# ruuda/robigo-luculenta

Hardware: AMD Instinct MI355X
Metric: Mrays/sec on built-in scene at 1920x1080 (higher is better)
Workload: dtype f32

## Files before the change

__graft_entry__.py:

```python
import os
import subprocess
import sys

ROOT = os.path.dirname(os.path.abspath(__file__))


def _make(directory):
    subprocess.run(["make", "-C", os.path.join(ROOT, directory)], check=True)


def build():
    _make("robigo_luculenta_amd/csrc")
    _make("oracle")
    _make("tests/host_mirror")
    _make("tests/lds_poison")
    _make("examples")
    if ROOT not in sys.path:
        sys.path.insert(0, ROOT)
    import robigo_luculenta_amd


def smoke():
    if ROOT not in sys.path:
        sys.path.insert(0, ROOT)
    sys.path.insert(0, os.path.join(ROOT, "tests"))
    import numpy as np

    import robigo_luculenta_amd as R
    import _oracle as O

    assert R.device_count() > 0, "smoke() needs a GPU"
    W, H, N = 256, 144, 16384
    objs, cam = R.builtin_scene_desc(R.SCENE_DEMO)
    scene = R.Scene(objs, cam, device=0)
    trace = R.TraceUnit(0, W, H, n_photons=N)
    trace.render(scene, seed=1, stream=0, first_path_index=0)
    got = trace.mapped_photons
    want, segs = O.Scene(objs.view(O.OBJECT_DTYPE), O.RlCameraDesc.from_buffer_copy(bytes(cam))).render(W, H, 1, 0, 0, N, threads=4)
    assert got.tobytes() == want.tobytes(), "GPU photons differ from the CPU oracle"
    paths, segments, ms = trace.stats()
    assert (paths, segments) == (N, segs), (paths, segments, N, segs)
    plot = R.PlotUnit(0, W, H)
    plot.plot([trace])
    gather = R.GatherUnit(W, H)
    gather.accumulate(plot)
    tm = R.TonemapUnit(W, H)
    tm.tonemap(gather)
    rgb = tm.rgb_buffer
    ref_rgb, _, _ = O.tonemap(gather.tristimulus_buffer, W, H)
    assert np.abs(rgb.astype(int) - ref_rgb.astype(int)).max() <= 1
    print("smoke ok: %d photons bit-equal to the oracle, %d segments, %.3f ms kernel" % (N, segments, ms))


if __name__ == "__main__":
    build()
    if len(sys.argv) > 1 and sys.argv[1] == "smoke":
        smoke()
```

robigo_luculenta_amd/csrc/rl_scene.cpp:

```cpp
#include "rl_scene.h"

#include <algorithm>
#include <array>
#include <cmath>
#include <cstdio>
#include <cstdlib>
#include <cstring>
#include <limits>
#include <numeric>

#include "rl_core.h"

namespace {

const float PI = RL_PI_F;

RlVector3 V(float x, float y, float z) {
    RlVector3 v;
    v.x = x; v.y = y; v.z = z;
    return v;
}
RlVector3 V(RlF3 f) { return V(f.x, f.y, f.z); }
RlF3 F(const RlVector3& v) { return rl_f3(v.x, v.y, v.z); }
RlF4 F4(RlF3 v, float w) {
// ... 50 lines not shown
    for (int i = 0; i < count; ++i) {
        for (int v = 0; v < 2; ++v) {
            const float ofs = variants[v][0], radius = variants[v][1], phi_ofs = variants[v][2], h = variants[v][3];
            const float phi = (float)i * prism_angle + ofs;
            RlF3 position = rl_f3(rl_cosf_d(phi) * prism_radius * radius, rl_sinf_d(phi) * prism_radius * radius, 0.0f);
            RlF3 normal = rl_f3(0, 0, -1.0f);
            const float t = rl_paraboloid_t(floor.offset, floor.normal, floor.focal_point, position, normal);
            if (!(t < 0.0f)) {
                const RlF3 pos = rl_add(position, rl_mul(normal, t));
                const RlF3 local_pos = rl_sub(pos, floor.offset);
                const RlF3 plane_pr = rl_sub(local_pos, rl_mul(floor.normal, rl_dot(local_pos, floor.normal)));
                const RlF3 surface_normal = rl_normalise(rl_sub(floor.focal_point, plane_pr));
                normal = rl_neg(surface_normal);
                position = rl_add(pos, rl_mul(rl_mul(normal, 2.0f), h));
            }
            out.push_back(make_object(RL_SURFACE_HEX_PRISM, V(normal), V(position), 3.0f, 1.0f, phi + phi_ofs, prism_height * h,
                                      RL_MATERIAL_SF10_GLASS, 0, 0, 0));
        }
    }
}

RlCameraDesc demo_camera() {
    RlCameraDesc c;
    c.phi0 = 1.0f; c.phi1 = 0.01f;
    c.alpha0 = 0.3f; c.alpha1 = -0.01f;
    c.dist0 = 50.0f; c.dist1 = -0.5f;
    c.fov_over_pi = 0.35f;
    c.focal_factor = 0.9f;
    c.depth_of_field = 2.0f;
    c.chromatic_abberation = 0.012f;
    return c;
}

void demo_scene(int seeds, std::vector<RlObjectDesc>& out) {
    const float sun_radius = 5.0f;
    push_fixed_objects(out, sun_radius);
    const double golden_ratio = 1.6180339887498948482045868343656381177203091798057628;
    const float gamma = PI * 2.0f * (1.0f - 1.0f / (float)golden_ratio);
    const float seed_size = 0.8f, seed_scale = 1.5f;
    const float fs = sun_radius / seed_scale + 1.0f;
    const int first_seed = (int)(fs * fs + 0.5f);
    for (int i = first_seed; i < first_seed + seeds; ++i) {
        const float phi = (float)i * gamma;
        const float r = sqrtf((float)i) * seed_scale;
        const RlF3 c = rl_add(rl_f3(rl_cosf_d(phi) * r, rl_sinf_d(phi) * r, (r - sun_radius) * -0.5f), rl_f3(0, 0, 0));
        out.push_back(sphere(c, seed_size, RL_MATERIAL_DIFFUSE_COLOURED, 0.9f,
                             (float)(i - first_seed) / (float)seeds * 130.0f + 600.0f, 60.0f));
    }
    for (int i = first_seed; i < first_seed + seeds; ++i) {
        const float fi = (float)i + 0.5f;
        const float phi = fi * gamma;
        const float r = sqrtf(fi) * seed_scale;
        const RlF3 c = rl_add(rl_f3(rl_cosf_d(phi) * r, rl_sinf_d(phi) * r, (r - sun_radius) * -0.25f), rl_f3(0, 0, 0));
        out.push_back(sphere(c, seed_size * 0.5f, RL_MATERIAL_GLOSSY_MIRROR, 0.1f));
    }
    for (int i = first_seed / 2; i < first_seed + seeds; ++i) {
        const float phi = (float)(-i) * gamma;
        const float root = sqrtf((float)i);
        const float r = root * seed_scale * 1.5f;
        const RlF3 c = rl_add(rl_f3(rl_cosf_d(phi) * r, rl_sinf_d(phi) * r, (r - sun_radius) * 1.5f + sun_radius * 2.0f), rl_f3(0, 0, 0));
        out.push_back(sphere(c, seed_size * (0.5f + root * 0.2f), RL_MATERIAL_SOAP_BUBBLE));
    }
    push_prism_ring(out, sun_radius, 11, 17.0f);
}

void glass_stress_scene(std::vector<RlObjectDesc>& out) {
    const float sun_radius = 5.0f;
    push_fixed_objects(out, sun_radius);
    push_prism_ring(out, sun_radius, 11, 10.0f);
    push_prism_ring(out, sun_radius, 11, 17.0f);
    push_prism_ring(out, sun_radius, 11, 24.0f);
}

void push_infinite_prism(std::vector<RlF4>& recs, RlF3 axis, RlF3 offset, float edge_length, float angle, float objbits) {
    const float radius = sqrtf(3.0f) / 6.0f * edge_length;
    const float a[3] = {angle, angle + PI * 2.0f / 3.0f, angle + PI * 4.0f / 3.0f};
    for (int k = 0; k < 3; ++k) {
        const RlF3 p = rl_rotate_towards(rl_f3(rl_cosf_d(a[k]), rl_sinf_d(a[k]), 0.0f), axis);
        recs.push_back(F4(p, 0.0f));
        recs.push_back(F4(rl_add(rl_mul(p, radius), offset), objbits));
    }
}

void prism_vertices(const RlF4* pr, std::vector<double>& vx, std::vector<double>& vy, std::vector<double>& vz) {
    double n[8][3], d[8];
    for (int k = 0; k < 8; ++k) {
        n[k][0] = pr[2 * k].x; n[k][1] = pr[2 * k].y; n[k][2] = pr[2 * k].z;
        d[k] = n[k][0] * pr[2 * k + 1].x + n[k][1] * pr[2 * k + 1].y + n[k][2] * pr[2 * k + 1].z;
    }
    for (int a = 0; a < 8; ++a)
        for (int b = a + 1; b < 8; ++b)
            for (int c = b + 1; c < 8; ++c) {
                const double* A = n[a]; const double* B = n[b]; const double* Cc = n[c];
                const double bxc[3] = {B[1] * Cc[2] - B[2] * Cc[1], B[2] * Cc[0] - B[0] * Cc[2], B[0] * Cc[1] - B[1] * Cc[0]};
                const double cxa[3] = {Cc[1] * A[2] - Cc[2] * A[1], Cc[2] * A[0] - Cc[0] * A[2], Cc[0] * A[1] - Cc[1] * A[0]};
                const double axb[3] = {A[1] * B[2] - A[2] * B[1], A[2] * B[0] - A[0] * B[2], A[0] * B[1] - A[1] * B[0]};
                const double det = A[0] * bxc[0] + A[1] * bxc[1] + A[2] * bxc[2];
                if (std::fabs(det) < 1e-9) continue;
                double p[3];
                for (int i = 0; i < 3; ++i) p[i] = (d[a] * bxc[i] + d[b] * cxa[i] + d[c] * axb[i]) / det;
                bool inside = true;
                for (int k = 0; k < 8 && inside; ++k)
                    inside = (n[k][0] * p[0] + n[k][1] * p[1] + n[k][2] * p[2] - d[k]) <= 1e-6;
                if (inside) {
                    vx.push_back(p[0]); vy.push_back(p[1]); vz.push_back(p[2]);
                }
            }
}

RlF4 prism_bound(const RlF4* pr) {
    std::vector<double> vx, vy, vz;
    prism_vertices(pr, vx, vy, vz);
    bool unbounded = false;
    RlF4 r;
    r.x = r.y = r.z = 0.0f;
    r.w = std::numeric_limits<float>::infinity();
    if (vx.size() < 4) return r;
    double c[3] = {0, 0, 0};
    for (size_t i = 0; i < vx.size(); ++i) { c[0] += vx[i]; c[1] += vy[i]; c[2] += vz[i]; }
    for (int i = 0; i < 3; ++i) c[i] /= (double)vx.size();
    double r2 = 0;
    for (size_t i = 0; i < vx.size(); ++i) {
        const double dx = vx[i] - c[0], dy = vy[i] - c[1], dz = vz[i] - c[2];
        r2 = std::max(r2, dx * dx + dy * dy + dz * dz);
    }
    if (!(r2 < 1e12)) unbounded = true;
    if (unbounded) return r;
    const double radius = std::sqrt(r2) * 1.05 + 1e-3;
    r.x = (float)c[0]; r.y = (float)c[1]; r.z = (float)c[2];
    r.w = (float)(radius * radius);
    return r;
}

void prism_cylinder(const RlF4* pr, RlF4 out[2]) {
    out[0] = RlF4{0.0f, 0.0f, 0.0f, std::numeric_limits<float>::infinity()};
    out[1] = RlF4{0.0f, 0.0f, 1.0f, 0.0f};
    std::vector<double> vx, vy, vz;
    prism_vertices(pr, vx, vy, vz);
    double a[3] = {pr[14].x, pr[14].y, pr[14].z};
    const double al = std::sqrt(a[0] * a[0] + a[1] * a[1] + a[2] * a[2]);
    if (vx.size() < 4 || !(al > 1e-12)) return;
    for (double& v : a) v /= al;
    double c[3] = {0, 0, 0};
    for (size_t i = 0; i < vx.size(); ++i) { c[0] += vx[i]; c[1] += vy[i]; c[2] += vz[i]; }
    for (double& v : c) v /= (double)vx.size();
    double r2 = 0;
    for (size_t i = 0; i < vx.size(); ++i) {
        const double d[3] = {vx[i] - c[0], vy[i] - c[1], vz[i] - c[2]};
        const double along = d[0] * a[0] + d[1] * a[1] + d[2] * a[2];
        r2 = std::max(r2, d[0] * d[0] + d[1] * d[1] + d[2] * d[2] - along * along);
    }
    if (!(r2 < 1e12)) return;
    out[0] = RlF4{(float)c[0], (float)c[1], (float)c[2], (float)(std::sqrt(std::max(r2, 0.0)) * 1.05 + 1e-3)};
    out[1] = RlF4{(float)a[0], (float)a[1], (float)a[2], 0.0f};
}

struct SphereIn {
    RlF4 rec;
    uint32_t obj;
    double radius;
};

void split_clusters(const std::vector<SphereIn>& sph, std::vector<uint32_t> idx, std::vector<std::vector<uint32_t>>& out, size_t K) {
    if (idx.size() <= K) {
        if (!idx.empty()) out.push_back(idx);
        return;
    }
    double lo[3] = {1e300, 1e300, 1e300}, hi[3] = {-1e300, -1e300, -1e300};
    for (uint32_t i : idx) {
        const double c[3] = {sph[i].rec.x, sph[i].rec.y, sph[i].rec.z};
        for (int a = 0; a < 3; ++a) {
            lo[a] = std::min(lo[a], c[a]);
            hi[a] = std::max(hi[a], c[a]);
        }
    }
    int axis = 0;
    for (int a = 1; a < 3; ++a)
        if (hi[a] - lo[a] > hi[axis] - lo[axis]) axis = a;
    auto coord = [&](uint32_t i) { return axis == 0 ? sph[i].rec.x : axis == 1 ? sph[i].rec.y : sph[i].rec.z; };
    std::sort(idx.begin(), idx.end(), [&](uint32_t a, uint32_t b) { return coord(a) < coord(b) || (coord(a) == coord(b) && a < b); });
    size_t left = ((idx.size() / 2 + K - 1) / K) * K;
    if (left >= idx.size()) left = idx.size() - K;
    split_clusters(sph, std::vector<uint32_t>(idx.begin(), idx.begin() + left), out, K);
    split_clusters(sph, std::vector<uint32_t>(idx.begin() + left, idx.end()), out, K);
}

void refine_clusters(const std::vector<SphereIn>& sph, std::vector<std::vector<uint32_t>>& clusters, size_t K) {
    const size_t k = clusters.size();
    if (k < 2) return;
    std::vector<uint32_t> all;
    for (const auto& c : clusters) all.insert(all.end(), c.begin(), c.end());
    std::sort(all.begin(), all.end());
    for (int iteration = 0; iteration < 24; ++iteration) {
        std::vector<double> cx(k, 0), cy(k, 0), cz(k, 0);
        for (size_t j = 0; j < k; ++j) {
            for (uint32_t i : clusters[j]) {
                cx[j] += sph[i].rec.x; cy[j] += sph[i].rec.y; cz[j] += sph[i].rec.z;
            }
            const double n = (double)std::max<size_t>(1, clusters[j].size());
            cx[j] /= n; cy[j] /= n; cz[j] /= n;
        }
        auto dist2 = [&](uint32_t i, size_t j) {
            const double dx = sph[i].rec.x - cx[j], dy = sph[i].rec.y - cy[j], dz = sph[i].rec.z - cz[j];
            return dx * dx + dy * dy + dz * dz;
        };
        std::vector<std::pair<double, uint32_t>> order;
        for (uint32_t i : all) {
            double best = 1e300, second = 1e300;
            for (size_t j = 0; j < k; ++j) {
                const double d = dist2(i, j);
                if (d < best) { second = best; best = d; }
                else if (d < second) second = d;
            }
            order.push_back({std::sqrt(best) - std::sqrt(second), i});
        }
        std::sort(order.begin(), order.end());
        std::vector<std::vector<uint32_t>> next(k);
        for (const auto& entry : order) {
            const uint32_t i = entry.second;
            size_t pick = k;
            double pick_d = 1e300;
            for (size_t j = 0; j < k; ++j) {
                if (next[j].size() >= K) continue;
                const double d = dist2(i, j);
                if (d < pick_d) { pick_d = d; pick = j; }
            }
            next[pick].push_back(i);
        }
        bool same = true;
        for (size_t j = 0; j < k && same; ++j) {
            std::sort(next[j].begin(), next[j].end());
            std::vector<uint32_t> old = clusters[j];
            std::sort(old.begin(), old.end());
            same = old == next[j];
        }
        clusters = next;
        if (same) break;
// ... 35 lines not shown
    return radius * radius;
}
void improve_partition(const std::vector<Ball>& items, std::vector<std::vector<uint32_t>>& bins, size_t capacity) {
    const size_t k = bins.size();
    if (k < 2) return;
    for (const Ball& b : items)
        if (!(b.r < 1e15)) return;
    const size_t NEIGHBOURS = 6, CANDIDATES = 3, PARTNERS = 4;
    std::vector<double> r2(k);
    std::vector<std::array<double, 3>> centre(k);
    auto refresh = [&](size_t j) {
        r2[j] = bin_radius2(items, bins[j]);
        std::array<double, 3> c = {0, 0, 0};
        for (uint32_t i : bins[j])
            for (int a = 0; a < 3; ++a) c[a] += items[i].c[a];
        for (int a = 0; a < 3; ++a) c[a] /= (double)std::max<size_t>(1, bins[j].size());
        centre[j] = c;
    };
    for (size_t j = 0; j < k; ++j) refresh(j);
    auto outermost = [&](size_t j, size_t count) {
        std::vector<std::pair<double, uint32_t>> by_reach;
        for (uint32_t i : bins[j]) {
            double d2 = 0;
            for (int a = 0; a < 3; ++a) d2 += (items[i].c[a] - centre[j][a]) * (items[i].c[a] - centre[j][a]);
            by_reach.push_back({-(std::sqrt(d2) + items[i].r), i});
        }
        std::sort(by_reach.begin(), by_reach.end());
        std::vector<uint32_t> out;
        for (size_t n = 0; n < by_reach.size() && n < count; ++n) out.push_back(by_reach[n].second);
        return out;
    };
    auto without = [](std::vector<uint32_t> v, uint32_t i) {
        v.erase(std::find(v.begin(), v.end(), i));
        return v;
    };
    const int passes = k <= 256 ? 8 : k <= 1024 ? 3 : 1;
    for (int pass = 0; pass < passes; ++pass) {
        bool improved = false;
        for (size_t a = 0; a < k; ++a) {
            if (bins[a].size() < 2) continue;
            for (uint32_t i : outermost(a, CANDIDATES)) {
                std::vector<std::pair<double, size_t>> near;
                for (size_t b = 0; b < k; ++b) {
                    if (b == a || bins[b].empty()) continue;
                    double d2 = 0;
                    for (int x = 0; x < 3; ++x) d2 += (items[i].c[x] - centre[b][x]) * (items[i].c[x] - centre[b][x]);
                    near.push_back({d2, b});
                }
                std::sort(near.begin(), near.end());
                double best_gain = 1e-9 * (r2[a] + 1.0);
                size_t best_b = k;
                std::vector<uint32_t> best_a_members, best_b_members;
                const std::vector<uint32_t> a_less = without(bins[a], i);
                for (size_t n = 0; n < near.size() && n < NEIGHBOURS; ++n) {
                    const size_t b = near[n].second;
                    const double before = r2[a] + r2[b];
                    if (bins[b].size() < capacity) {
                        std::vector<uint32_t> b_more = bins[b];
                        b_more.push_back(i);
                        const double gain = before - (bin_radius2(items, a_less) + bin_radius2(items, b_more));
                        if (gain > best_gain) { best_gain = gain; best_b = b; best_a_members = a_less; best_b_members = b_more; }
                    }
                    for (uint32_t j : outermost(b, PARTNERS)) {
                        std::vector<uint32_t> a_new = a_less, b_new = without(bins[b], j);
                        a_new.push_back(j);
                        b_new.push_back(i);
                        const double gain = before - (bin_radius2(items, a_new) + bin_radius2(items, b_new));
                        if (gain > best_gain) { best_gain = gain; best_b = b; best_a_members = a_new; best_b_members = b_new; }
                    }
                }
                if (best_b == k) continue;
                bins[a] = best_a_members;
                bins[best_b] = best_b_members;
                refresh(a);
                refresh(best_b);
                improved = true;
                break;
            }
        }
        if (!improved) break;
    }
}

RlF4 cluster_bound(const std::vector<SphereIn>& sph, const std::vector<uint32_t>& members) {
    double c[3] = {0, 0, 0};
    for (uint32_t i : members) {
        c[0] += sph[i].rec.x; c[1] += sph[i].rec.y; c[2] += sph[i].rec.z;
    }
    for (int a = 0; a < 3; ++a) c[a] /= (double)members.size();
    auto reach = [&](uint32_t i) {
        const double dx = sph[i].rec.x - c[0], dy = sph[i].rec.y - c[1], dz = sph[i].rec.z - c[2];
        return std::sqrt(dx * dx + dy * dy + dz * dz) + sph[i].radius;
    };
    for (int it = 0; it < 64; ++it) {
        uint32_t far = members[0];
        for (uint32_t i : members)
            if (reach(i) > reach(far)) far = i;
        const double step = 0.5 / (it + 2.0);
        c[0] += (sph[far].rec.x - c[0]) * step; c[1] += (sph[far].rec.y - c[1]) * step; c[2] += (sph[far].rec.z - c[2]) * step;
    }
    double radius = 0;
    for (uint32_t i : members) radius = std::max(radius, reach(i));
    radius = radius * 1.05 + 0.05;
    RlF4 b;
    b.x = (float)c[0]; b.y = (float)c[1]; b.z = (float)c[2];
    b.w = (float)(radius * radius);
    if (!(radius < 1e15)) b.w = std::numeric_limits<float>::infinity();
    return b;
}


double bound_radius(const RlF4& b) { return b.w > 0.0f ? std::sqrt((double)b.w) : 0.0; }

void split_groups(const std::vector<RlF4>& b, std::vector<uint32_t> idx, std::vector<std::vector<uint32_t>>& out, size_t G) {
    if (idx.size() <= G) {
        if (!idx.empty()) out.push_back(idx);
        return;
    }
    double lo[3] = {1e300, 1e300, 1e300}, hi[3] = {-1e300, -1e300, -1e300};
    for (uint32_t i : idx) {
        const double c[3] = {b[i].x, b[i].y, b[i].z};
        for (int a = 0; a < 3; ++a) {
            lo[a] = std::min(lo[a], c[a]);
            hi[a] = std::max(hi[a], c[a]);
        }
    }
    int axis = 0;
    for (int a = 1; a < 3; ++a)
        if (hi[a] - lo[a] > hi[axis] - lo[axis]) axis = a;
    auto coord = [&](uint32_t i) { return axis == 0 ? b[i].x : axis == 1 ? b[i].y : b[i].z; };
    std::sort(idx.begin(), idx.end(), [&](uint32_t p, uint32_t q) { return coord(p) < coord(q) || (coord(p) == coord(q) && p < q); });
    size_t left = ((idx.size() / 2 + G - 1) / G) * G;
    if (left >= idx.size()) left = idx.size() - G;
    split_groups(b, std::vector<uint32_t>(idx.begin(), idx.begin() + left), out, G);
    split_groups(b, std::vector<uint32_t>(idx.begin() + left, idx.end()), out, G);
}

void refine_groups(const std::vector<RlF4>& b, std::vector<std::vector<uint32_t>>& groups, size_t G) {
    const size_t k = groups.size();
    if (k < 2) return;
    std::vector<uint32_t> all;
    for (const auto& g : groups) all.insert(all.end(), g.begin(), g.end());
    std::sort(all.begin(), all.end());
    for (int iteration = 0; iteration < 24; ++iteration) {
        std::vector<double> cx(k, 0), cy(k, 0), cz(k, 0);
        for (size_t j = 0; j < k; ++j) {
            for (uint32_t i : groups[j]) {
                cx[j] += b[i].x; cy[j] += b[i].y; cz[j] += b[i].z;
            }
            const double n = (double)std::max<size_t>(1, groups[j].size());
            cx[j] /= n; cy[j] /= n; cz[j] /= n;
        }
        auto dist2 = [&](uint32_t i, size_t j) {
            const double dx = b[i].x - cx[j], dy = b[i].y - cy[j], dz = b[i].z - cz[j];
            return dx * dx + dy * dy + dz * dz;
        };
        std::vector<std::pair<double, uint32_t>> order;
        for (uint32_t i : all) {
            double best = 1e300, second = 1e300;
            for (size_t j = 0; j < k; ++j) {
                const double d = dist2(i, j);
                if (d < best) { second = best; best = d; }
                else if (d < second) second = d;
            }
            order.push_back({std::sqrt(best) - std::sqrt(second), i});
        }
        std::sort(order.begin(), order.end());
        std::vector<std::vector<uint32_t>> next(k);
        for (const auto& entry : order) {
            const uint32_t i = entry.second;
            size_t pick = k;
            double pick_d = 1e300;
            for (size_t j = 0; j < k; ++j) {
                if (next[j].size() >= G) continue;
                const double d = dist2(i, j);
                if (d < pick_d) { pick_d = d; pick = j; }
            }
            next[pick].push_back(i);
        }
        bool same = true;
        for (size_t j = 0; j < k && same; ++j) {
            std::sort(next[j].begin(), next[j].end());
            std::vector<uint32_t> old = groups[j];
            std::sort(old.begin(), old.end());
            same = old == next[j];
        }
        groups = next;
        if (same) break;
    }
    std::vector<std::vector<uint32_t>> kept;
    for (auto& g : groups)
        if (!g.empty()) kept.push_back(g);
    groups = kept;
}

RlF4 group_bound(const std::vector<RlF4>& b, const std::vector<uint32_t>& members) {
    RlF4 r;
    r.x = r.y = r.z = 0.0f;
    r.w = std::numeric_limits<float>::infinity();
    for (uint32_t i : members)
        if (!(b[i].w < 1e30f)) return r;
    double c[3] = {0, 0, 0};
    for (uint32_t i : members) {
        c[0] += b[i].x; c[1] += b[i].y; c[2] += b[i].z;
    }
    for (int a = 0; a < 3; ++a) c[a] /= (double)members.size();
    auto reach = [&](uint32_t i) {
        const double dx = b[i].x - c[0], dy = b[i].y - c[1], dz = b[i].z - c[2];
        return std::sqrt(dx * dx + dy * dy + dz * dz) + bound_radius(b[i]);
    };
    for (int it = 0; it < 64; ++it) {
        uint32_t far = members[0];
        for (uint32_t i : members)
            if (reach(i) > reach(far)) far = i;
        const double step = 0.5 / (it + 2.0);
        c[0] += (b[far].x - c[0]) * step; c[1] += (b[far].y - c[1]) * step; c[2] += (b[far].z - c[2]) * step;
    }
    r.x = (float)c[0]; r.y = (float)c[1]; r.z = (float)c[2];
    c[0] = r.x; c[1] = r.y; c[2] = r.z;
    double radius = 0;
    for (uint32_t i : members) radius = std::max(radius, reach(i));
    radius = radius * 1.001 + 1e-3;
    r.w = (float)(radius * radius);
    if (!(radius < 1e15)) r.w = std::numeric_limits<float>::infinity();
    return r;
}

std::vector<uint32_t> order_by_groups(const std::vector<RlF4>& bounds, std::vector<std::vector<uint32_t>>* groups_out, size_t G) {
    std::vector<uint32_t> idx(bounds.size());
    std::iota(idx.begin(), idx.end(), 0u);
    std::vector<std::vector<uint32_t>> groups;
    split_groups(bounds, idx, groups, G);
    refine_groups(bounds, groups, G);
    {
        std::vector<Ball> balls;
        for (const RlF4& b : bounds) balls.push_back(Ball{{b.x, b.y, b.z}, bound_radius(b)});
        improve_partition(balls, groups, G);
    }
    std::vector<uint32_t> order;
    for (std::vector<uint32_t>& g : groups) {
        std::sort(g.begin(), g.end());
        order.insert(order.end(), g.begin(), g.end());
    }
    *groups_out = groups;
    return order;
}

constexpr uint32_t RL_SUPER_MIN_GROUPS = 112;
constexpr uint32_t RL_SUPER_G_DEFAULT = 8;
void super_params(uint32_t* min_groups, uint32_t* sg) {
    *min_groups = RL_SUPER_MIN_GROUPS;
    *sg = RL_SUPER_G_DEFAULT;
    if (const char* e = std::getenv("RL_SUPER_MIN")) *min_groups = (uint32_t)std::max(1, std::atoi(e));
    if (const char* e = std::getenv("RL_SUPER_G")) *sg = (uint32_t)std::min(64, std::max(2, std::atoi(e)));
}
struct ClusterPlan {
    uint32_t k, group_gc;
    std::vector<std::vector<uint32_t>> clusters;
    std::vector<RlF4> cluster_bounds, group_bounds;
    double cost;
};

ClusterPlan plan_clusters(const std::vector<SphereIn>& sph, const std::vector<std::vector<uint32_t>>& clusters, uint32_t k, uint32_t group_gc) {
    ClusterPlan plan;
    plan.k = k;
    plan.group_gc = group_gc;
    plan.cost = 0;
    std::vector<RlF4> bounds;
    for (const std::vector<uint32_t>& members : clusters) bounds.push_back(cluster_bound(sph, members));
    std::vector<std::vector<uint32_t>> groups;
    order_by_groups(bounds, &groups, group_gc);
    const RlF4 never = RlF4{0.0f, 0.0f, 0.0f, -std::numeric_limits<float>::infinity()};
    for (const std::vector<uint32_t>& g : groups) {
        std::vector<RlF4> members;
        std::vector<uint32_t> all(g.size());
        for (uint32_t k2 : g) {
            plan.clusters.push_back(clusters[k2]);
            plan.cluster_bounds.push_back(bounds[k2]);
            members.push_back(bounds[k2]);
        }
        std::iota(all.begin(), all.end(), 0u);
        plan.group_bounds.push_back(group_bound(members, all));
        for (size_t pad = g.size(); pad < group_gc; ++pad) {
            plan.clusters.push_back(std::vector<uint32_t>());
            plan.cluster_bounds.push_back(never);
        }
    }
    return plan;
}

std::vector<RlF4> sample_path_rays(const RlFlatScene& fs, const std::vector<SphereIn>& sph) {
    std::vector<RlF4> spheres, objects = fs.objects;
    std::vector<uint32_t> sphere_obj;
    for (const SphereIn& si : sph) {
        objects[si.obj].w = rl_u2f(rl_object_bits(rl_object_surface(rl_f2u(objects[si.obj].w)), rl_object_material(rl_f2u(objects[si.obj].w)), (uint32_t)spheres.size()));
        spheres.push_back(si.rec);
        sphere_obj.push_back(si.obj);
    }
    RlSceneView sv;
    std::memset(&sv, 0, sizeof sv);
    sv.spheres = spheres.data();
    sv.sphere_obj = sphere_obj.data();
    sv.objects = objects.data();
    sv.planes = fs.planes.data();
    sv.parabs = fs.parabs.data();
    sv.prisms = fs.prisms.data();
    sv.n_direct = sv.n_direct_padded = sv.cluster_base = (uint32_t)spheres.size();
    sv.n_planes = (uint32_t)(fs.planes.size() / 2);
    sv.n_parabs = (uint32_t)(fs.parabs.size() / 3);
    sv.n_prisms = (uint32_t)(fs.prisms.size() / RL_PRISM_STRIDE);
    sv.n_objects = (uint32_t)objects.size();
    sv.camera_rec = fs.camera_rec.data();
    RlSceneView flat_things = sv;
    flat_things.n_direct = 0;
    flat_things.n_prisms = 0;
    std::vector<RlF4> rays;
    const uint64_t seed = 0x706c616e6e696e67ull;
    for (uint64_t path = 0; path < 384 && rays.size() < 2 * 2048; ++path) {
        RlPath p;
        rl_begin_path(sv, 16.0f / 9.0f, seed, 0u, path, &p);
        for (int bounce = 0; bounce < 64; ++bounce) {
            const RlHit nearest_flat = rl_scan(flat_things, p.origin, p.direction);
            rays.push_back(RlF4{p.origin.x, p.origin.y, p.origin.z, nearest_flat.t * 1.0002f});
            rays.push_back(RlF4{p.direction.x, p.direction.y, p.direction.z, 0.0f});
            const RlHit hit = rl_scan(sv, p.origin, p.direction);
            float value = 0.0f;
            uint32_t emitter = 0;
            if (rl_bounce(sv, seed, 0u, path, &p, hit, &value, &emitter) != RL_PATH_CONTINUES) break;
        }
    }
    return rays;
}

double plan_cost(const ClusterPlan& plan, const std::vector<RlF4>& rays) {
    auto reaches = [](const RlF4& b, const RlF4& o, const RlF4& d) {
        if (!(b.w > 0.0f)) return false;
        const double cx = (double)b.x - o.x, cy = (double)b.y - o.y, cz = (double)b.z - o.z;
        const double d2 = (double)d.x * d.x + (double)d.y * d.y + (double)d.z * d.z;
        const double along = std::min(std::max(0.0, (cx * d.x + cy * d.y + cz * d.z) / d2), (double)o.w);
        const double px = cx - along * d.x, py = cy - along * d.y, pz = cz - along * d.z;
        return px * px + py * py + pz * pz <= (double)b.w;
    };
    const double n_rays = (double)(rays.size() / 2);
    uint32_t min_groups, sg;
    super_params(&min_groups, &sg);
    const size_t n_groups = plan.group_bounds.size();
    std::vector<std::vector<uint32_t>> supers;
    std::vector<RlF4> super_bounds;
    if (n_groups >= min_groups && n_groups > sg) {
        order_by_groups(plan.group_bounds, &supers, sg);
        for (const std::vector<uint32_t>& members : supers) super_bounds.push_back(group_bound(plan.group_bounds, members));
    } else {
        supers.assign(1, std::vector<uint32_t>());
        for (uint32_t g = 0; g < n_groups; ++g) supers[0].push_back(g);
    }
    double super_pairs = 0, group_pairs = 0, cluster_pairs = 0;
    for (size_t r = 0; r + 1 < rays.size(); r += 2) {
        for (size_t s = 0; s < supers.size(); ++s) {
            if (!super_bounds.empty()) {
                if (!reaches(super_bounds[s], rays[r], rays[r + 1])) continue;
                super_pairs += 1;
            }
            for (uint32_t g : supers[s]) {
                if (!reaches(plan.group_bounds[g], rays[r], rays[r + 1])) continue;
                group_pairs += 1;
                for (size_t k = plan.group_gc * g; k < plan.group_gc * (g + 1); ++k)
                    if (reaches(plan.cluster_bounds[k], rays[r], rays[r + 1])) cluster_pairs += 1;
            }
        }
    }
    const double top = super_bounds.empty() ? 0.59 * (double)n_groups
                                            : 0.59 * (double)super_bounds.size() + super_pairs / n_rays * (2.3 + 0.9 * (double)sg);
    const double cost = top + group_pairs / n_rays * (2.13 + 0.83 * ((double)plan.group_gc - 3.0)) +
                        cluster_pairs / n_rays * (0.25 + 0.40 * plan.k);
    return cost;
}

}

uint32_t rl_builtin_scene(int which, int param, std::vector<RlObjectDesc>* out, RlCameraDesc* camera) {
    std::vector<RlObjectDesc> objs;
    if (which == RL_SCENE_DEMO) demo_scene(param > 0 ? param : 100, objs);
    else if (which == RL_SCENE_GLASS_STRESS) glass_stress_scene(objs);
    else return 0;
    if (camera) *camera = demo_camera();
    if (out) *out = objs;
    return (uint32_t)objs.size();
}

static void set_group(RlF4& object, uint32_t group_index) {
    const uint32_t bits = rl_f2u(object.w);
    object.w = rl_u2f(rl_object_bits(rl_object_surface(bits), rl_object_material(bits), group_index));
}

int rl_flatten_scene(const RlSceneDesc* desc, RlFlatScene* out, const char** err) {
    *err = "";
    if (!desc || (!desc->objects && desc->n_objects)) {
        *err = "null scene description";
        return RL_E_INVALID;
    }
    if (desc->n_objects > (1u << 24)) {
        *err = "more than 2^24 objects";
        return RL_E_INVALID;
    }
    RlFlatScene& fs = *out;
    fs = RlFlatScene();
    std::vector<SphereIn> sph_in;
    fs.camera = desc->camera;
    const float fov = PI * desc->camera.fov_over_pi;
    fs.screen_distance = 1.0f / rl_tanf(fov * 0.5f);
    fs.camera_rec.assign(3, RlF4{0.0f, 0.0f, 0.0f, 0.0f});
    std::memcpy(fs.camera_rec.data(), &fs.camera, sizeof(RlCameraDesc));
    reinterpret_cast<float*>(fs.camera_rec.data())[10] = fs.screen_distance;
    for (uint32_t i = 0; i < desc->n_objects; ++i) {
        const RlObjectDesc& o = desc->objects[i];
        const float objbits = rl_u2f(i);
        uint32_t group_index = 0;
        switch (o.surface_kind) {
        case RL_SURFACE_SPHERE: {
            SphereIn si;
            si.rec = F4(F(o.v0), o.f0 * o.f0);
            si.obj = i;
            si.radius = std::fabs((double)o.f0);
            sph_in.push_back(si);
            group_index = 0;
            break;
        }
        case RL_SURFACE_PLANE:
        case RL_SURFACE_CIRCLE:
            group_index = (uint32_t)(fs.planes.size() / 2);
            fs.planes.push_back(F4(F(o.v0), o.surface_kind == RL_SURFACE_CIRCLE ? o.f0 * o.f0 : -1.0f));
            fs.planes.push_back(F4(F(o.v1), objbits));
            break;
        case RL_SURFACE_PARABOLOID: {
// ... 114 lines not shown
    }
    fs.cluster_k = plan.k;
    fs.group_gc = plan.group_gc;
    {
        uint32_t min_groups, sg;
        super_params(&min_groups, &sg);
        const size_t n_groups = plan.clusters.size() / plan.group_gc;
        if (n_groups >= min_groups && n_groups > sg) {
            std::vector<std::vector<uint32_t>> supers;
            order_by_groups(plan.group_bounds, &supers, sg);
            std::vector<std::vector<uint32_t>> ordered;
            for (const std::vector<uint32_t>& members : supers) {
                for (uint32_t g : members)
                    for (uint32_t c = 0; c < plan.group_gc; ++c) ordered.push_back(plan.clusters[(size_t)plan.group_gc * g + c]);
                for (size_t pad = members.size(); pad < sg; ++pad)
                    for (uint32_t c = 0; c < plan.group_gc; ++c) ordered.push_back(std::vector<uint32_t>());
            }
            plan.clusters = ordered;
            fs.n_cluster_supers = (uint32_t)supers.size();
            fs.super_g = sg;
        }
    }
    const RlF4 never = dummy;
    std::vector<std::vector<uint32_t>>& clusters = plan.clusters;
    for (std::vector<uint32_t>& members : clusters) {
        std::sort(members.begin(), members.end());
        fs.spheres.push_back(members.empty() ? never : cluster_bound(sph_in, members));
        fs.sphere_obj.push_back(RL_HIT_NONE);
        for (uint32_t k : members) place(k);
        for (size_t pad = members.size(); pad < fs.cluster_k; ++pad) {
            fs.spheres.push_back(dummy);
            fs.sphere_obj.push_back(RL_HIT_NONE);
        }
    }
    fs.n_clusters = (uint32_t)clusters.size();
    fs.n_cluster_groups = fs.n_clusters / fs.group_gc;
    uint32_t n_prisms = (uint32_t)(fs.prisms.size() / RL_PRISM_STRIDE);
    if (n_prisms != 0) {
        std::vector<RlF4> bounds;
        for (uint32_t i = 0; i < n_prisms; ++i) bounds.push_back(fs.prisms[RL_PRISM_STRIDE * i + 16]);
        std::vector<std::vector<uint32_t>> groups;
        order_by_groups(bounds, &groups, RL_GROUP_GP);
        std::vector<RlF4> sorted;
        for (const std::vector<uint32_t>& g : groups) {
            for (uint32_t k : g) {
                const RlF4* pr = &fs.prisms[RL_PRISM_STRIDE * k];
                set_group(fs.objects[rl_f2u(pr[1].w)], (uint32_t)(sorted.size() / RL_PRISM_STRIDE));
                sorted.insert(sorted.end(), pr, pr + RL_PRISM_STRIDE);
            }
            for (size_t pad = g.size(); pad < RL_GROUP_GP; ++pad) {
                sorted.resize(sorted.size() + RL_PRISM_STRIDE - 1, RlF4{0.0f, 0.0f, 0.0f, 0.0f});
                sorted.push_back(never);
            }
        }
        fs.prisms = sorted;
        n_prisms = (uint32_t)(fs.prisms.size() / RL_PRISM_STRIDE);
    }
    fs.n_prism_groups = n_prisms / RL_GROUP_GP;
    uint32_t real_prisms = 0;
    fs.prism_cyl.clear();
    for (uint32_t i = 0; i < n_prisms; ++i) {
        RlF4 cyl[2];
        prism_cylinder(&fs.prisms[RL_PRISM_STRIDE * i], cyl);
        fs.prism_cyl.push_back(cyl[0]);
        fs.prism_cyl.push_back(cyl[1]);
        if (std::isfinite(fs.prisms[RL_PRISM_STRIDE * i + 16].w) && fs.prisms[RL_PRISM_STRIDE * i + 16].w > 0.0f) real_prisms += 1;
    }
    fs.prism_cylinders = real_prisms >= 40u;
    if (!fs.prism_cylinders) fs.prism_cyl.clear();
    fs.cull_cmax2 = 0.0f;
    auto add_bound = [&](const RlF4& b) {
        const double c2 = (double)b.x * b.x + (double)b.y * b.y + (double)b.z * b.z;
        RlF4 r = b;
        r.w = (float)(c2 - (double)b.w);
        fs.cull_bounds.push_back(r);
        if (std::isfinite(b.w)) fs.cull_cmax2 = std::max(fs.cull_cmax2, (float)c2 * 1.0001f);
    };
    std::vector<RlF4> level1;
    for (uint32_t k = 0; k < fs.n_clusters; ++k) level1.push_back(fs.spheres[fs.cluster_base + (fs.cluster_k + 1u) * k]);
    for (uint32_t i = 0; i < n_prisms; ++i) level1.push_back(fs.prisms[RL_PRISM_STRIDE * i + 16]);
    for (const RlF4& b : level1) add_bound(b);
    const size_t n_cluster_level1 = (size_t)fs.group_gc * fs.n_cluster_groups;
    std::vector<RlF4> level2;
    for (size_t first = 0; first < level1.size();) {
        const size_t G = first < n_cluster_level1 ? fs.group_gc : RL_GROUP_GP;
        std::vector<uint32_t> members;
        for (size_t j = first; j < first + G; ++j)
            if (!(level1[j].w == never.w)) members.push_back((uint32_t)j);
        level2.push_back(members.empty() ? never : group_bound(level1, members));
        add_bound(level2.back());
        first += G;
    }
    for (uint32_t s = 0; s < fs.n_cluster_supers; ++s) {
        std::vector<uint32_t> members;
        for (uint32_t g = fs.super_g * s; g < fs.super_g * (s + 1u); ++g)
            if (!(level2[g].w == never.w)) members.push_back(g);
        add_bound(members.empty() ? never : group_bound(level2, members));
    }
    fs.cull_bounds.push_back(dummy);
    fs.cull_bounds.push_back(dummy);
    {
        uint32_t last_parab = 0, first_plane = 0xffffffffu;
        for (size_t i = 0; i < fs.parabs.size(); i += 3) last_parab = std::max(last_parab, rl_f2u(fs.parabs[i].w));
        for (size_t i = 1; i < fs.planes.size(); i += 2) first_plane = std::min(first_plane, rl_f2u(fs.planes[i].w));
        bool sorted = fs.parabs.empty() || fs.planes.empty() || last_parab < first_plane;
        for (size_t i = 3; i < fs.parabs.size(); i += 3) sorted = sorted && rl_f2u(fs.parabs[i - 3].w) < rl_f2u(fs.parabs[i].w);
        for (size_t i = 3; i < fs.planes.size(); i += 2) sorted = sorted && rl_f2u(fs.planes[i - 2].w) < rl_f2u(fs.planes[i].w);
        fs.small_ordered = sorted;
        bool axis_z = !(fs.parabs.empty() && fs.planes.empty());
        for (size_t i = 1; i < fs.parabs.size(); i += 3) axis_z = axis_z && fs.parabs[i].x == 0.0f && fs.parabs[i].y == 0.0f;
        for (size_t i = 0; i < fs.planes.size(); i += 2) axis_z = axis_z && fs.planes[i].x == 0.0f && fs.planes[i].y == 0.0f;
        fs.small_axis_z = axis_z;
    }
    fs.sphere_cull_w.assign(fs.spheres.size(), std::numeric_limits<float>::infinity());
    for (size_t pos = fs.cluster_base; pos < fs.spheres.size(); ++pos) {
        const RlF4& sp = fs.spheres[pos];
        if (fs.sphere_obj[pos] == RL_HIT_NONE || !std::isfinite(sp.w) || !(sp.w >= 0.0f)) continue;
        const double c2 = (double)sp.x * sp.x + (double)sp.y * sp.y + (double)sp.z * sp.z;
        fs.sphere_cull_w[pos] = (float)(c2 - ((double)sp.w * 1.001 + 1.0e-6));
        fs.cull_cmax2 = std::max(fs.cull_cmax2, (float)c2 * 1.0001f);
    }
    return RL_OK;
}
```

Baseline: 22940.

## Tighten culling bounds with exact minimum enclosing balls and error-aware padding

Replaces the centroid/iterative approximate bounding spheres for prisms, prism cylinders, clusters, groups and supers with a minimum-enclosing-ball solver that enumerates support sets of up to four items. The fixed 5% plus constant slack is replaced by a small relative pad plus a drift pad derived from float error, with radii rounded up to float. Tighter bounds should reject more ray/bound pairs in the hierarchical cull and so cut intersection work per ray. The cost is extra host-side scene-build time and a risk of culling correctness if the padding underestimates float error.

```diff
diff --git a/__graft_entry__.py b/__graft_entry__.py
--- a/__graft_entry__.py
+++ b/__graft_entry__.py
@@ -13,6 +13,7 @@
     _make("robigo_luculenta_amd/csrc")
     _make("oracle")
     _make("tests/host_mirror")
+    _make("tests/cull_slack")
     _make("tests/lds_poison")
     _make("examples")
     if ROOT not in sys.path:
diff --git a/robigo_luculenta_amd/csrc/rl_scene.cpp b/robigo_luculenta_amd/csrc/rl_scene.cpp
--- a/robigo_luculenta_amd/csrc/rl_scene.cpp
+++ b/robigo_luculenta_amd/csrc/rl_scene.cpp
@@ -156,6 +156,139 @@
     }
 }
 
+constexpr double RL_BOUND_REL = 1.0e-4, RL_BOUND_POS = 1.0e-6, RL_BOUND_EPS = 1.021e-4, RL_BOUND_KAPPA = 9.0e-4;
+constexpr double RL_BOUND_PAD_MAX = 1.07;
+double drift_pad(double R, double r_min) {
+    const double u = RL_BOUND_EPS * R / (RL_BOUND_KAPPA - RL_BOUND_EPS);
+    return r_min < u ? (u - r_min) * (u - r_min) / (2.0 * u) : 0.0;
+}
+float round_up(double v) {
+    const float f = (float)v;
+    return (double)f < v ? std::nextafterf(f, std::numeric_limits<float>::infinity()) : f;
+}
+
+struct BallItem {
+    double c[3], r;
+};
+constexpr size_t MIN_BALL_SUPPORT = 8;
+double ball_reach(const std::vector<BallItem>& items, const double c[3]) {
+    double reach = 0;
+    for (const BallItem& b : items) {
+        const double dx = b.c[0] - c[0], dy = b.c[1] - c[1], dz = b.c[2] - c[2];
+        reach = std::max(reach, std::sqrt(dx * dx + dy * dy + dz * dz) + b.r);
+    }
+    return reach;
+}
+double padded_reach(const std::vector<BallItem>& spheres, const double c[3], double R_upper) {
+    double reach = 0;
+    for (const BallItem& b : spheres) {
+        const double dx = b.c[0] - c[0], dy = b.c[1] - c[1], dz = b.c[2] - c[2];
+        reach = std::max(reach, std::sqrt(dx * dx + dy * dy + dz * dz) + b.r + drift_pad(R_upper, b.r));
+    }
+    return reach;
+}
+void min_ball_centre(const std::vector<BallItem>& items, double centre[3]) {
+    const size_t n = items.size();
+    double c[3] = {0, 0, 0};
+    for (const BallItem& b : items)
+        for (int a = 0; a < 3; ++a) c[a] += b.c[a] / (double)n;
+    auto reach_of = [&](size_t i, const double at[3]) {
+        const double dx = items[i].c[0] - at[0], dy = items[i].c[1] - at[1], dz = items[i].c[2] - at[2];
+        return std::sqrt(dx * dx + dy * dy + dz * dz) + items[i].r;
+    };
+    for (int it = 0; it < 64; ++it) {
+        size_t far = 0;
+        for (size_t i = 1; i < n; ++i)
+            if (reach_of(i, c) > reach_of(far, c)) far = i;
+        const double step = 0.5 / (it + 2.0);
+        for (int a = 0; a < 3; ++a) c[a] += (items[far].c[a] - c[a]) * step;
+    }
+    double best = ball_reach(items, c);
+    for (int a = 0; a < 3; ++a) centre[a] = c[a];
+    if (!(best < 1e15)) return;
+    std::vector<std::pair<double, size_t>> by_reach;
+    for (size_t i = 0; i < n; ++i) by_reach.push_back({-reach_of(i, c), i});
+    std::sort(by_reach.begin(), by_reach.end());
+    const size_t m = std::min(n, MIN_BALL_SUPPORT);
+    auto consider = [&](const double at[3]) {
+        if (!(std::isfinite(at[0]) && std::isfinite(at[1]) && std::isfinite(at[2]))) return;
+        const double reach = ball_reach(items, at);
+        if (reach < best) {
+            best = reach;
+            for (int a = 0; a < 3; ++a) centre[a] = at[a];
+        }
+    };
+    for (uint32_t mask = 1; mask < (1u << m); ++mask) {
+        const int k = __builtin_popcount(mask);
+        if (k > 4) continue;
+        const BallItem* s[4];
+        int cnt = 0;
+        for (size_t j = 0; j < m; ++j)
+            if (mask & (1u << j)) s[cnt++] = &items[by_reach[j].second];
+        if (k == 1) {
+            consider(s[0]->c);
+            continue;
+        }
+        const int d = k - 1;
+        double e[3][3], G[3][3], p[3], q[3];
+        for (int j = 0; j < d; ++j) {
+            for (int a = 0; a < 3; ++a) e[j][a] = s[j + 1]->c[a] - s[0]->c[a];
+            p[j] = 0.5 * (e[j][0] * e[j][0] + e[j][1] * e[j][1] + e[j][2] * e[j][2] - s[j + 1]->r * s[j + 1]->r + s[0]->r * s[0]->r);
+            q[j] = s[j + 1]->r - s[0]->r;
+        }
+        double scale = 0;
+        for (int i = 0; i < d; ++i)
+            for (int j = 0; j < d; ++j) {
+                G[i][j] = e[i][0] * e[j][0] + e[i][1] * e[j][1] + e[i][2] * e[j][2];
+                if (i == j) scale = std::max(scale, G[i][j]);
+            }
+        double M[3][5];
+        for (int i = 0; i < d; ++i) {
+            for (int j = 0; j < d; ++j) M[i][j] = G[i][j];
+            M[i][d] = p[i];
+            M[i][d + 1] = q[i];
+        }
+        bool singular = false;
+        for (int col = 0; col < d && !singular; ++col) {
+            int piv = col;
+            for (int i = col + 1; i < d; ++i)
+                if (std::fabs(M[i][col]) > std::fabs(M[piv][col])) piv = i;
+            if (!(std::fabs(M[piv][col]) > 1e-12 * scale)) { singular = true; break; }
+            for (int j = 0; j < d + 2; ++j) std::swap(M[col][j], M[piv][j]);
+            for (int i = 0; i < d; ++i) {
+                if (i == col) continue;
+                const double f = M[i][col] / M[col][col];
+                for (int j = col; j < d + 2; ++j) M[i][j] -= f * M[col][j];
+            }
+        }
+        if (singular) continue;
+        double u[3] = {0, 0, 0}, v[3] = {0, 0, 0};
+        for (int j = 0; j < d; ++j) {
+            const double A = M[j][d] / M[j][j], B = M[j][d + 1] / M[j][j];
+            for (int a = 0; a < 3; ++a) { u[a] += A * e[j][a]; v[a] += B * e[j][a]; }
+        }
+        const double r0 = s[0]->r;
+        const double qa = v[0] * v[0] + v[1] * v[1] + v[2] * v[2] - 1.0, qb = 2.0 * (u[0] * v[0] + u[1] * v[1] + u[2] * v[2] + r0),
+                     qc = u[0] * u[0] + u[1] * u[1] + u[2] * u[2] - r0 * r0;
+        double roots[2];
+        int n_roots = 0;
+        if (std::fabs(qa) < 1e-14) {
+            if (std::fabs(qb) > 0) roots[n_roots++] = -qc / qb;
+        } else {
+            const double disc = qb * qb - 4.0 * qa * qc;
+            if (disc >= 0) {
+                roots[n_roots++] = (-qb + std::sqrt(disc)) / (2.0 * qa);
+                roots[n_roots++] = (-qb - std::sqrt(disc)) / (2.0 * qa);
+            }
+        }
+        for (int t = 0; t < n_roots; ++t) {
+            if (!(roots[t] >= r0)) continue;
+            const double at[3] = {s[0]->c[0] + u[0] + roots[t] * v[0], s[0]->c[1] + u[1] + roots[t] * v[1], s[0]->c[2] + u[2] + roots[t] * v[2]};
+            consider(at);
+        }
+    }
+}
+
 void prism_vertices(const RlF4* pr, std::vector<double>& vx, std::vector<double>& vy, std::vector<double>& vz) {
     double n[8][3], d[8];
     for (int k = 0; k < 8; ++k) {
@@ -190,19 +323,18 @@
     r.x = r.y = r.z = 0.0f;
     r.w = std::numeric_limits<float>::infinity();
     if (vx.size() < 4) return r;
-    double c[3] = {0, 0, 0};
-    for (size_t i = 0; i < vx.size(); ++i) { c[0] += vx[i]; c[1] += vy[i]; c[2] += vz[i]; }
-    for (int i = 0; i < 3; ++i) c[i] /= (double)vx.size();
-    double r2 = 0;
-    for (size_t i = 0; i < vx.size(); ++i) {
-        const double dx = vx[i] - c[0], dy = vy[i] - c[1], dz = vz[i] - c[2];
-        r2 = std::max(r2, dx * dx + dy * dy + dz * dz);
-    }
-    if (!(r2 < 1e12)) unbounded = true;
+    std::vector<BallItem> items;
+    for (size_t i = 0; i < vx.size(); ++i) items.push_back(BallItem{{vx[i], vy[i], vz[i]}, 0.0});
+    double c[3];
+    min_ball_centre(items, c);
+    const float cf[3] = {(float)c[0], (float)c[1], (float)c[2]};
+    for (int i = 0; i < 3; ++i) c[i] = cf[i];
+    const double reach = ball_reach(items, c);
+    if (!(reach * reach < 1e12)) unbounded = true;
     if (unbounded) return r;
-    const double radius = std::sqrt(r2) * 1.05 + 1e-3;
-    r.x = (float)c[0]; r.y = (float)c[1]; r.z = (float)c[2];
-    r.w = (float)(radius * radius);
+    const double radius = reach * (1.0 + RL_BOUND_REL) + RL_BOUND_POS * (std::sqrt(c[0] * c[0] + c[1] * c[1] + c[2] * c[2]) + reach);
+    r.x = cf[0]; r.y = cf[1]; r.z = cf[2];
+    r.w = round_up(radius * radius);
     return r;
 }
 
@@ -214,19 +346,31 @@
     double a[3] = {pr[14].x, pr[14].y, pr[14].z};
     const double al = std::sqrt(a[0] * a[0] + a[1] * a[1] + a[2] * a[2]);
     if (vx.size() < 4 || !(al > 1e-12)) return;
-    for (double& v : a) v /= al;
-    double c[3] = {0, 0, 0};
-    for (size_t i = 0; i < vx.size(); ++i) { c[0] += vx[i]; c[1] += vy[i]; c[2] += vz[i]; }
-    for (double& v : c) v /= (double)vx.size();
+    const float af[3] = {(float)(a[0] / al), (float)(a[1] / al), (float)(a[2] / al)};
+    const double afl = std::sqrt((double)af[0] * af[0] + (double)af[1] * af[1] + (double)af[2] * af[2]);
+    for (int i = 0; i < 3; ++i) a[i] = (double)af[i] / afl;
+    double mean[3] = {0, 0, 0};
+    for (size_t i = 0; i < vx.size(); ++i) { mean[0] += vx[i]; mean[1] += vy[i]; mean[2] += vz[i]; }
+    for (double& v : mean) v /= (double)vx.size();
+    std::vector<BallItem> flat;
+    for (size_t i = 0; i < vx.size(); ++i) {
+        const double d[3] = {vx[i] - mean[0], vy[i] - mean[1], vz[i] - mean[2]};
+        const double along = d[0] * a[0] + d[1] * a[1] + d[2] * a[2];
+        flat.push_back(BallItem{{d[0] - along * a[0], d[1] - along * a[1], d[2] - along * a[2]}, 0.0});
+    }
+    double c[3];
+    min_ball_centre(flat, c);
+    const float cf[3] = {(float)(c[0] + mean[0]), (float)(c[1] + mean[1]), (float)(c[2] + mean[2])};
     double r2 = 0;
     for (size_t i = 0; i < vx.size(); ++i) {
-        const double d[3] = {vx[i] - c[0], vy[i] - c[1], vz[i] - c[2]};
+        const double d[3] = {vx[i] - cf[0], vy[i] - cf[1], vz[i] - cf[2]};
         const double along = d[0] * a[0] + d[1] * a[1] + d[2] * a[2];
         r2 = std::max(r2, d[0] * d[0] + d[1] * d[1] + d[2] * d[2] - along * along);
     }
     if (!(r2 < 1e12)) return;
-    out[0] = RlF4{(float)c[0], (float)c[1], (float)c[2], (float)(std::sqrt(std::max(r2, 0.0)) * 1.05 + 1e-3)};
-    out[1] = RlF4{(float)a[0], (float)a[1], (float)a[2], 0.0f};
+    const double radius = std::sqrt(std::max(r2, 0.0)) * 1.05 + 1e-3;
+    out[0] = RlF4{cf[0], cf[1], cf[2], round_up(radius)};
+    out[1] = RlF4{af[0], af[1], af[2], 0.0f};
 }
 
 struct SphereIn {
@@ -428,29 +572,18 @@
     }
 }
 
+BallItem ball_of(const SphereIn& s) { return BallItem{{s.rec.x, s.rec.y, s.rec.z}, std::max(s.radius, s.rec.w > 0.0f ? std::sqrt((double)s.rec.w) : 0.0)}; }
 RlF4 cluster_bound(const std::vector<SphereIn>& sph, const std::vector<uint32_t>& members) {
-    double c[3] = {0, 0, 0};
-    for (uint32_t i : members) {
-        c[0] += sph[i].rec.x; c[1] += sph[i].rec.y; c[2] += sph[i].rec.z;
-    }
-    for (int a = 0; a < 3; ++a) c[a] /= (double)members.size();
-    auto reach = [&](uint32_t i) {
-        const double dx = sph[i].rec.x - c[0], dy = sph[i].rec.y - c[1], dz = sph[i].rec.z - c[2];
-        return std::sqrt(dx * dx + dy * dy + dz * dz) + sph[i].radius;
-    };
-    for (int it = 0; it < 64; ++it) {
-        uint32_t far = members[0];
-        for (uint32_t i : members)
-            if (reach(i) > reach(far)) far = i;
-        const double step = 0.5 / (it + 2.0);
-        c[0] += (sph[far].rec.x - c[0]) * step; c[1] += (sph[far].rec.y - c[1]) * step; c[2] += (sph[far].rec.z - c[2]) * step;
-    }
-    double radius = 0;
-    for (uint32_t i : members) radius = std::max(radius, reach(i));
-    radius = radius * 1.05 + 0.05;
+    std::vector<BallItem> items;
+    for (uint32_t i : members) items.push_back(ball_of(sph[i]));
+    double c[3];
+    min_ball_centre(items, c);
     RlF4 b;
     b.x = (float)c[0]; b.y = (float)c[1]; b.z = (float)c[2];
-    b.w = (float)(radius * radius);
+    c[0] = b.x; c[1] = b.y; c[2] = b.z;
+    const double reach = ball_reach(items, c);
+    const double radius = padded_reach(items, c, reach * RL_BOUND_PAD_MAX) * (1.0 + RL_BOUND_REL);
+    b.w = round_up(radius * radius);
     if (!(radius < 1e15)) b.w = std::numeric_limits<float>::infinity();
     return b;
 }
@@ -540,34 +673,21 @@
     groups = kept;
 }
 
-RlF4 group_bound(const std::vector<RlF4>& b, const std::vector<uint32_t>& members) {
+RlF4 group_bound(const std::vector<RlF4>& b, const std::vector<uint32_t>& members, const std::vector<BallItem>& spheres) {
     RlF4 r;
     r.x = r.y = r.z = 0.0f;
     r.w = std::numeric_limits<float>::infinity();
     for (uint32_t i : members)
         if (!(b[i].w < 1e30f)) return r;
-    double c[3] = {0, 0, 0};
-    for (uint32_t i : members) {
-        c[0] += b[i].x; c[1] += b[i].y; c[2] += b[i].z;
-    }
-    for (int a = 0; a < 3; ++a) c[a] /= (double)members.size();
-    auto reach = [&](uint32_t i) {
-        const double dx = b[i].x - c[0], dy = b[i].y - c[1], dz = b[i].z - c[2];
-        return std::sqrt(dx * dx + dy * dy + dz * dz) + bound_radius(b[i]);
-    };
-    for (int it = 0; it < 64; ++it) {
-        uint32_t far = members[0];
-        for (uint32_t i : members)
-            if (reach(i) > reach(far)) far = i;
-        const double step = 0.5 / (it + 2.0);
-        c[0] += (b[far].x - c[0]) * step; c[1] += (b[far].y - c[1]) * step; c[2] += (b[far].z - c[2]) * step;
-    }
+    std::vector<BallItem> items;
+    for (uint32_t i : members) items.push_back(BallItem{{b[i].x, b[i].y, b[i].z}, bound_radius(b[i])});
+    double c[3];
+    min_ball_centre(items, c);
     r.x = (float)c[0]; r.y = (float)c[1]; r.z = (float)c[2];
     c[0] = r.x; c[1] = r.y; c[2] = r.z;
-    double radius = 0;
-    for (uint32_t i : members) radius = std::max(radius, reach(i));
-    radius = radius * 1.001 + 1e-3;
-    r.w = (float)(radius * radius);
+    const double reach = ball_reach(items, c);
+    const double radius = std::max(reach, padded_reach(spheres, c, reach * RL_BOUND_PAD_MAX)) * (1.0 + RL_BOUND_REL);
+    r.w = round_up(radius * radius);
     if (!(radius < 1e15)) r.w = std::numeric_limits<float>::infinity();
     return r;
 }
@@ -605,6 +725,7 @@
     std::vector<std::vector<uint32_t>> clusters;
     std::vector<RlF4> cluster_bounds, group_bounds;
     double cost;
+    std::vector<std::vector<BallItem>> group_spheres;
 };
 
 ClusterPlan plan_clusters(const std::vector<SphereIn>& sph, const std::vector<std::vector<uint32_t>>& clusters, uint32_t k, uint32_t group_gc) {
@@ -620,13 +741,16 @@
     for (const std::vector<uint32_t>& g : groups) {
         std::vector<RlF4> members;
         std::vector<uint32_t> all(g.size());
+        std::vector<BallItem> below;
         for (uint32_t k2 : g) {
+            for (uint32_t i : clusters[k2]) below.push_back(ball_of(sph[i]));
             plan.clusters.push_back(clusters[k2]);
             plan.cluster_bounds.push_back(bounds[k2]);
             members.push_back(bounds[k2]);
         }
         std::iota(all.begin(), all.end(), 0u);
-        plan.group_bounds.push_back(group_bound(members, all));
+        plan.group_bounds.push_back(group_bound(members, all, below));
+        plan.group_spheres.push_back(below);
         for (size_t pad = g.size(); pad < group_gc; ++pad) {
             plan.clusters.push_back(std::vector<uint32_t>());
             plan.cluster_bounds.push_back(never);
@@ -695,7 +819,11 @@
     std::vector<RlF4> super_bounds;
     if (n_groups >= min_groups && n_groups > sg) {
         order_by_groups(plan.group_bounds, &supers, sg);
-        for (const std::vector<uint32_t>& members : supers) super_bounds.push_back(group_bound(plan.group_bounds, members));
+        for (const std::vector<uint32_t>& members : supers) {
+            std::vector<BallItem> below;
+            for (uint32_t g : members) below.insert(below.end(), plan.group_spheres[g].begin(), plan.group_spheres[g].end());
+            super_bounds.push_back(group_bound(plan.group_bounds, members, below));
+        }
     } else {
         supers.assign(1, std::vector<uint32_t>());
         for (uint32_t g = 0; g < n_groups; ++g) supers[0].push_back(g);
@@ -976,12 +1104,19 @@
     for (const RlF4& b : level1) add_bound(b);
     const size_t n_cluster_level1 = (size_t)fs.group_gc * fs.n_cluster_groups;
     std::vector<RlF4> level2;
+    std::vector<std::vector<BallItem>> level2_spheres;
     for (size_t first = 0; first < level1.size();) {
         const size_t G = first < n_cluster_level1 ? fs.group_gc : RL_GROUP_GP;
         std::vector<uint32_t> members;
-        for (size_t j = first; j < first + G; ++j)
-            if (!(level1[j].w == never.w)) members.push_back((uint32_t)j);
-        level2.push_back(members.empty() ? never : group_bound(level1, members));
+        std::vector<BallItem> below;
+        for (size_t j = first; j < first + G; ++j) {
+            if (level1[j].w == never.w) continue;
+            members.push_back((uint32_t)j);
+            if (j < n_cluster_level1)
+                for (uint32_t i : clusters[j]) below.push_back(ball_of(sph_in[i]));
+        }
+        level2.push_back(members.empty() ? never : group_bound(level1, members, below));
+        level2_spheres.push_back(below);
         add_bound(level2.back());
         first += G;
     }
@@ -989,7 +1124,9 @@
         std::vector<uint32_t> members;
         for (uint32_t g = fs.super_g * s; g < fs.super_g * (s + 1u); ++g)
             if (!(level2[g].w == never.w)) members.push_back(g);
-        add_bound(members.empty() ? never : group_bound(level2, members));
+        std::vector<BallItem> below;
+        for (uint32_t g : members) below.insert(below.end(), level2_spheres[g].begin(), level2_spheres[g].end());
+        add_bound(members.empty() ? never : group_bound(level2, members, below));
     }
     fs.cull_bounds.push_back(dummy);
     fs.cull_bounds.push_back(dummy);
```

Result: no change. 23160 (median of 6 runs) (+1.0%).
